# mmdagent/distantspeechrecognition-mirror

Measured on AMD Instinct MI355X. Metric: decoded_audio_hours_per_sec, higher is better.
Workload: dtype f32

## Files before the change

distantspeechrecognition-mirror_amd/csrc/decoder.cpp:

```cpp
#include "common.h"
#include "wfst_graph.h"
#include "lattice.h"
#include "lexicon.h"
#include "wordtrace.h"
#include "viterbi.h"
#include "decode_plan.h"
#include <algorithm>
#include <cmath>

namespace dsr {

static_assert(kPlanSideBytes == (size_t) kSideLds * sizeof(Side), "decode_plan.h budgets the side records of viterbi.h");

struct DecoderState {
  dsr_decoder_cfg cfg; bool haveGraph = false; int nSlots = 0; int nNodes = 0;
  WfstGraph::Csr csr; WfstGraph::Tables tab;
  DevBuf<int> d_xoff, d_xarc, d_xpathOff, d_eoff, d_path, d_nodeFinal, d_queue; DevBuf<float> d_pathCost;
  DevBuf<XRec> d_xrec; DevBuf<ERec> d_erec; DevBuf<float> d_arcCost, d_nodeCost; DevBuf<uint32_t> d_arcOut, d_arcIn;
  DevBuf<TokA> d_tokA, d_ctok; DevBuf<TokB> d_tokB; DevBuf<Side> d_side; DevBuf<XRecD> d_xrecD; int fastOK = 0; int maxCnt = 0; DevBuf<int> d_tokOff, d_tokCnt, d_owner, d_rank, d_chead; DevBuf<unsigned> d_tags; DevBuf<CandA> d_cA; DevBuf<CandB> d_cB; DevBuf<unsigned> d_first; DevBuf<Bp> d_arena;
  DevBuf<long long> d_prof; DevBuf<dsr_decode_result> d_res; DevBuf<int> d_arcs; DevBuf<unsigned> d_words;
  long arenaCap = 0; int initial = 0; unsigned tokenMemoryLimit = 0;
  long lastPoolCap = 0;
  hipEvent_t evTrace = nullptr;
  DevBuf<TraceHead> d_heads; DevBuf<int> d_hopRec, d_hopOff;
  DevBuf<SegState> d_segState; DevBuf<int> d_segDone; DevBuf<unsigned long long> d_poolNext; DevBuf<TokA> d_saveA; DevBuf<TokB> d_saveB;
  DevBuf<WTok> w_tok; DevBuf<WCand> w_cand; DevBuf<int> w_tokOff, w_rank; DevBuf<unsigned long long> w_best; DevBuf<unsigned> w_first; DevBuf<int4> w_traces; size_t w_tablesFor = 0;
  bool costNegZero = false; double costMinAbs = HUGE_VAL;
  DevBuf<uint4> d_lat; DevBuf<double> d_latTtl; DevBuf<long> d_latFrameOff; DevBuf<int> d_arenaLat; DevBuf<int4> d_latFinal; DevBuf<int> d_latInfo;
  int latU = 0, latTmax = 0; long latArenaCap = 0; WfstGraph graphCopy; DevBuf<TokA> d_tokA3; DevBuf<TokB> d_tokB3;
  const dsr_lexicon* lexIn = nullptr; const dsr_lexicon* lexOut = nullptr; uint32_t eosX = 0; std::string eosSymbol;
  int lastU = 0; size_t lastMaxPath = 0; bool lastPaths = false;
  PinBuf<dsr_decode_result> h_res; PinBuf<int> h_arcs; PinBuf<unsigned> h_words; hipEvent_t evDone = nullptr;
  int pendingU = 0; size_t pendingPath = 0; int pendingSlots = 0; long long* pendingProf = nullptr;
  int dumpOn = 0; long dumpCap = 0; DevBuf<long> d_dumpFrameOff, d_dumpCount; DevBuf<int> d_dumpNode, d_dumpArc; DevBuf<float> d_dumpAc, d_dumpLm;
  std::vector<int64_t> h_dumpFrameOff; std::vector<int32_t> h_dumpNode, h_dumpArc; std::vector<float> h_dumpAc, h_dumpLm; int64_t h_dumpFrames = 0;
};

}

using namespace dsr;
struct dsr_decoder : DecoderState {};

// ... 49 lines not shown

void dsr_decoder_destroy(dsr_decoder* d)
{
  if (!d) return;
  forget_traceback(d);
  if (d->evDone) (void) hipEventDestroy(d->evDone);
  if (d->evTrace) (void) hipEventDestroy(d->evTrace);
  delete d;
}

dsr_status dsr_decoder_set(dsr_decoder* d, const dsr_wfst* g)
{
  return guard([&] {
    if (!d || !g) throw Error(DSR_E_PARAMETER, "null argument");
    if (g->initial < 0) throw Error(DSR_E_CONSISTENCY, "the transducer has no arcs");
    d->csr = g->csr(); d->tab = g->tables(d->csr, (size_t) 1 << 28);
    d->nNodes = (int) g->nodes.size(); d->initial = g->initial; d->graphCopy = *g;
    std::vector<int> nf(d->nNodes); std::vector<float> nc(d->nNodes);
    for (int i = 0; i < d->nNodes; i++) { nf[i] = g->nodes[i].final_; nc[i] = g->nodes[i].cost; }
    d->d_xoff.upload(d->tab.xoff); d->d_eoff.upload(d->tab.eoff); d->d_path.upload(d->tab.path);
    if (d->tab.xrec.empty()) throw Error(DSR_E_CONSISTENCY, "the transducer has no emitting arcs");
    d->d_xrec.upload(d->tab.xrec); d->d_xarc.upload(d->tab.xarc); d->d_xpathOff.upload(d->tab.xpathOff);
    {
      const size_t nx = d->tab.xrec.size(); std::vector<XRecD> xd(nx); int maxCnt = 0; std::vector<float> pc(1, 0.0f);
      for (size_t r = 0; r < nx; r++) {
        const XRec& x = d->tab.xrec[r]; XRecD& o = xd[r];
        o.dst = x.dst; o.dist = x.dist; o.cost = x.cost; o.meta = x.meta; o.dstXoff = d->tab.xoff[x.dst]; o.dstCnt = d->tab.xoff[x.dst + 1] - d->tab.xoff[x.dst];
        const int po = d->tab.xpathOff[r], plen = (int) (x.meta & 0xFFFFu); o.p2 = 0; o.eps1 = 0.0f;
        if (x.meta >> 18) throw Error(DSR_E_CONSISTENCY, "expansion record %zu: meta bits above 17 are in use", r);
        if (plen) { const int a0 = d->tab.path[po]; o.eps1 = d->csr.cost[a0]; if (d->csr.out[a0] != 0) o.meta |= 0x20000u; }
        if (plen > 14) o.meta |= 0x80000000u;
        else if (plen > 1) {
          if (plen == 2) { const float c1 = d->csr.cost[d->tab.path[po + 1]]; memcpy(&o.p2, &c1, 4); }
          else { o.p2 = (int) pc.size(); for (int h = 1; h < plen; h++) pc.push_back(d->csr.cost[d->tab.path[po + h]]); }
          for (int h = 1; h < plen; h++) if (d->csr.out[d->tab.path[po + h]] != 0) o.meta |= 1u << (17 + h);
        }
        if (o.dstCnt > maxCnt) maxCnt = o.dstCnt;
      }
      d->d_xrecD.upload(xd); d->d_pathCost.upload(pc);
      d->fastOK = (maxCnt < (1 << 19) && nx < ((size_t) 1 << 27)) ? 1 : 0; d->maxCnt = maxCnt;
      if (read_vit_env().noFast) d->fastOK = 0;
    }
    { std::vector<ERec> e = d->tab.erec; if (e.empty()) e.push_back(ERec{0, 0, 0, 0}); d->d_erec.upload(e); }
    d->d_arcCost.upload(d->csr.cost); d->d_arcOut.upload(d->csr.out); d->d_arcIn.upload(d->csr.in);
    d->costNegZero = false; d->costMinAbs = HUGE_VAL;
    for (size_t a = 0; a < d->csr.cost.size(); a++) {
      const float c = d->csr.cost[a]; uint32_t bits; memcpy(&bits, &c, 4);
      if (bits == 0x80000000u) d->costNegZero = true;
      if (c != 0.0f && std::fabs((double) c) < d->costMinAbs) d->costMinAbs = std::fabs((double) c);
    }
    d->d_nodeFinal.upload(nf); d->d_nodeCost.upload(nc);
    d->haveGraph = true; d->nSlots = 0;
  });
}
dsr_status dsr_decoder_set_symbols(dsr_decoder* d, const dsr_wfst* g, const char* silSymbol, const char* eosSymbol)
{
  return guard([&] {
    if (!d || !g) throw Error(DSR_E_PARAMETER, "null argument");
    uint32_t silX = d->cfg.silenceX, eosX = 0;
    if (silSymbol) { if (!g->lexIn) throw Error(DSR_E_KEY, "the transducer has no input lexicon to look '%s' up in", silSymbol); silX = g->lexIn->index(silSymbol); }
    if (eosSymbol) { if (!g->lexOut) throw Error(DSR_E_KEY, "the transducer has no output lexicon to look '%s' up in", eosSymbol); eosX = g->lexOut->index(eosSymbol); }
    const dsr_status s = dsr_decoder_set(d, g);
// ... 145 lines not shown
  A.maxTok = c.maxActive; A.maxCand = c.maxCandidates; A.maxTraces = maxTraces;
  A.tok = d->w_tok.p; A.cand = d->w_cand.p; A.tokOff = d->w_tokOff.p; A.rank = d->w_rank.p; A.bestKey = d->w_best.p; A.firstSlot = d->w_first.p; A.traces = d->w_traces.p; A.queue = d->d_queue.p;
  A.scores = score; A.nframes = nframes; A.U = U; A.Tmax = Tmax; A.nDist = nDist; A.res = d->d_res.p; A.arcsOut = d->d_arcs.p; A.wordsOut = d->d_words.p; A.maxPath = maxPath;
  wordtrace_launch(A, slots, st);
  enqueue_result_copies(d, U, want_paths ? (size_t) U * maxPath : 0, st);
  d->pendingSlots = slots; d->pendingProf = nullptr; d->latU = 0;
}

static VitArgs fill_vit_args(dsr_decoder* d, const DecodePlan& P, const VitEnv& env, const float* score, const int32_t* nframes, int U, int Tmax, int nDist,
                             int maxPath, bool wantPaths, hipStream_t st)
{
  const int slots = P.slots; const bool latOn = d->cfg.latticeTokens > 0;
  d->d_res.reserve(U);
  if (wantPaths) { d->d_arcs.reserve((size_t) U * (maxPath > 0 ? maxPath : 1)); d->d_words.reserve((size_t) U * (maxPath > 0 ? maxPath : 1)); }
  DSR_HIP(hipMemsetAsync(d->d_queue.p, 0, 8 * sizeof(int), st));
  d->d_heads.reserve(U); DSR_HIP(hipMemsetAsync(d->d_heads.p, 0xFF, sizeof(TraceHead) * (size_t) U, st));
  if (d->dumpOn) {
    d->dumpCap = (long) d->cfg.maxActive * 64 < (long) 1 << 26 ? (long) 1 << 24 : (long) 1 << 26;
    d->d_dumpFrameOff.reserve(Tmax + 2); d->d_dumpCount.reserve(2);
    d->d_dumpNode.reserve(d->dumpCap); d->d_dumpArc.reserve(d->dumpCap); d->d_dumpAc.reserve(d->dumpCap); d->d_dumpLm.reserve(d->dumpCap);
    DSR_HIP(hipMemsetAsync(d->d_dumpCount.p, 0, 2 * sizeof(long), st));
  }
  VitArgs A; GraphDev& G = A.G; DecDev& D = A.D;
  G.nNodes = d->nNodes; G.initial = d->initial; G.xoff = d->d_xoff.p; G.xrec = d->d_xrec.p; G.xrecD = d->d_xrecD.p; G.xarc = d->d_xarc.p;
  G.xpathOff = d->d_xpathOff.p; G.eoff = d->d_eoff.p; G.erec = d->d_erec.p; G.path = d->d_path.p; G.pathCost = d->d_pathCost.p; G.arcCost = d->d_arcCost.p;
  G.arcOut = d->d_arcOut.p; G.arcIn = d->d_arcIn.p; G.nodeFinal = d->d_nodeFinal.p; G.nodeCost = d->d_nodeCost.p;
  D.beam = d->cfg.beam; D.lmScale = d->cfg.lmScale; D.lmPenalty = d->cfg.lmPenalty; D.silPenalty = d->cfg.silPenalty;
  D.noPen = (d->cfg.lmScale > 0.0 && std::isfinite(d->cfg.lmScale) && d->cfg.lmScale * d->cfg.lmPenalty == 0.0 && d->cfg.lmScale * d->cfg.silPenalty == 0.0 &&
             !d->costNegZero && (d->costMinAbs == HUGE_VAL || d->cfg.lmScale * d->costMinAbs >= 0x1p-60) && !env.pen) ? 1 : 0;
  D.silenceX = d->cfg.silenceX; D.maxTok = d->cfg.maxActive; D.maxCand = d->cfg.maxCandidates; D.arenaCap = d->arenaCap;
  D.tokA = d->d_tokA.p; D.tokB = d->d_tokB.p; D.ctok = d->d_ctok.p; D.side = d->d_side.p; D.fastOK = d->fastOK; D.tokOff = d->d_tokOff.p; D.owner = d->d_owner.p; D.rank = d->d_rank.p; D.cA = d->d_cA.p; D.cB = d->d_cB.p;
  D.first = d->d_first.p; D.tags = d->d_tags.p; D.tokCnt = d->d_tokCnt.p; D.chead = d->d_chead.p; D.arena = d->d_arena.p; D.queue = d->d_queue.p;
  D.segDrop = env.segDrop; D.segQueues = P.segQueues; D.segFrames = P.segFrames; D.segCount = P.segCount;
  D.poolCap = 0; D.poolChunk = 0; D.poolNext = nullptr; D.segState = nullptr; D.segDone = nullptr; D.saveA = nullptr; D.saveB = nullptr;
  if (P.segFrames > 0) {
    d->d_segState.reserve(U); d->d_segDone.reserve(U); d->d_poolNext.reserve(1);
    d->d_saveA.reserve((size_t) U * d->cfg.maxActive); d->d_saveB.reserve((size_t) U * d->cfg.maxActive);
    DSR_HIP(hipMemsetAsync(d->d_segDone.p, 0, sizeof(int) * (size_t) U, st)); DSR_HIP(hipMemsetAsync(d->d_poolNext.p, 0, sizeof(unsigned long long), st));
    D.poolCap = (long) ((size_t) std::max(P.poolArenas, slots) * (size_t) d->arenaCap); if (D.poolCap > (long) 0xFFFFFFF0L) D.poolCap = (long) 0xFFFFFFF0L;
    D.poolChunk = std::min<long>(262144, std::max<long>(4096, D.poolCap / (4 * (long) U)));
    D.poolNext = d->d_poolNext.p; D.segState = d->d_segState.p; D.segDone = d->d_segDone.p; D.saveA = d->d_saveA.p; D.saveB = d->d_saveB.p;
  }
  d->lastPoolCap = D.poolCap;
  D.prof = nullptr;
  if (env.prof) { d->d_prof.reserve((size_t) slots * kProfN); D.prof = d->d_prof.p; }
  D.dumpOn = d->dumpOn; D.dumpCap = d->dumpCap; D.dumpFrameOff = d->d_dumpFrameOff.p; D.dumpNode = d->d_dumpNode.p; D.dumpAc = d->d_dumpAc.p;
  D.dumpLm = d->d_dumpLm.p; D.dumpArc = d->d_dumpArc.p; D.dumpCount = d->d_dumpCount.p;
  D.topN = d->cfg.topN > 0 ? d->cfg.topN : 0; D.tokA3 = nullptr; D.tokB3 = nullptr;
  if (D.topN > 0) { d->d_tokA3.reserve((size_t) slots * d->cfg.maxActive); d->d_tokB3.reserve((size_t) slots * d->cfg.maxActive); D.tokA3 = d->d_tokA3.p; D.tokB3 = d->d_tokB3.p; }
// ... 254 lines not shown
```

distantspeechrecognition-mirror_amd/csrc/k_viterbi.hip:

```cpp
#include "launch.h"
#include "viterbi.h"
#include <algorithm>
#include <cmath>
#include <type_traits>

namespace dsr {

static constexpr uint32_t kNone = 0xFFFFFFFFu;
static constexpr uint32_t kEndBit = 0x80000000u;
static constexpr int kWaves = kThreads / 64;
static constexpr int kFastK = 8;
static constexpr int kB = 2;
static constexpr int kFastE = 8190;
static constexpr int kP1 = 16;
static constexpr int kW = 4;

typedef const __attribute__((address_space(4))) VitArgs* KP;

__device__ __forceinline__ unsigned ld_u32(const unsigned* p) { return __hip_atomic_load(p, __ATOMIC_RELAXED, __HIP_MEMORY_SCOPE_AGENT); }
__device__ __forceinline__ int ld_i32(const int* p) { return __hip_atomic_load(p, __ATOMIC_RELAXED, __HIP_MEMORY_SCOPE_AGENT); }
__device__ __forceinline__ void st_u32(unsigned* p, unsigned v) { __hip_atomic_store(p, v, __ATOMIC_RELAXED, __HIP_MEMORY_SCOPE_AGENT); }
__device__ __forceinline__ void st_i32(int* p, int v) { __hip_atomic_store(p, v, __ATOMIC_RELAXED, __HIP_MEMORY_SCOPE_AGENT); }
__device__ __forceinline__ void st_u64_dev(void* p, unsigned long long v) { __hip_atomic_store(reinterpret_cast<unsigned long long*>(p), v, __ATOMIC_RELAXED, __HIP_MEMORY_SCOPE_AGENT); }
__device__ __forceinline__ unsigned long long ld_u64_dev(const void* p) { return __hip_atomic_load(reinterpret_cast<const unsigned long long*>(p), __ATOMIC_RELAXED, __HIP_MEMORY_SCOPE_AGENT); }
// ... 376 lines not shown
            return atomicExch(&hkey[h], 0x80000000u | (unsigned) sx);
          };
          auto chain_head = [&](const unsigned h) __attribute__((always_inline)) -> unsigned {
            if (NARROW) { const unsigned w = tab[h]; return (w & 0x80000000u) ? (0x80000000u | ((w >> 15) & 0xFFFFu)) : 0u; }
            return hkey[h];
          };
          auto locate = [&](const int k, int& rec, unsigned& ekk) __attribute__((always_inline)) {
            const int c = k * nthr + tq; const int grp = k * nw + wq;
            unsigned e = 0u; int j = 0;
            if (c < C) {
              const unsigned long long W = ((unsigned long long) s_bm[2 * grp + 1] << 32) | s_bm[2 * grp];
              const unsigned gb = s_gbase[grp]; const unsigned long long mine = W & ((2ull << lq) - 1ull);
              e = (gb & 0x1FFFu) + (unsigned) __popcll(mine) - 1u;
              j = mine ? lq - (63 - __clzll((long long) mine)) : lq + (int) (gb >> 13);
            }
            ekk = e; rec = j;
          };
          auto tokload = [&](float& ac, float& lm, int& rec, unsigned& ekk) __attribute__((always_inline)) {
            const TokA t = *at32<TokA>(ctk, ekk * 16u);
            ac = t.ac; lm = t.lm; rec += (int) (t.xs & 0x7FFFFFFFu); ekk |= (t.xs >> 31) << 29;
          };
          auto expandR = [&](auto NOPEN, const int g8, float* ac8, float* lm8, int* rec8, unsigned* ek8) __attribute__((always_inline)) {
            constexpr bool NP = decltype(NOPEN)::value;
            int4 xr[kB]; int2 xd[kB]; bool tsil[kB];
#pragma unroll
            for (int i = 0; i < kB; i++) { tsil[i] = (ek8[i] >> 29) & 1u; ek8[i] &= 0x1FFFu; }
#pragma unroll
            for (int i = 0; i < kB; i++) {
              xr[i] = *at32<int4>(xrecD, (uint32_t) rec8[i] * 32u); xd[i] = *at32<int2>(xrecD, (uint32_t) rec8[i] * 32u + 16u);
            }
            if (PROF) { asm volatile("s_waitcnt vmcnt(0)" ::: "memory"); TICK(28); }
#pragma unroll
            for (int i = 0; i < kB; i++) {
              const int c = (g8 + i) * nthr + tq;
              if (c < C) {
                const int xdist = xr[i].x; const float xcost = __int_as_float(xr[i].y); const uint32_t xmeta = (uint32_t) xr[i].z;
                const float e1 = __int_as_float(xr[i].w);
                const int plen = (int) (xmeta & 0xFFFFu);
                const double lm0 = (double) lm8[i];
                const bool has = plen != 0;
                double lmNode;
                {
                  double l = __dadd_rn(lm0, __dmul_rn(lmS, (double) e1));
                  if (!NP) {
                    const double l1 = __dadd_rn(l, lsPen); l = (xmeta & 0x20000u) ? l1 : l;
                    const double l2 = __dadd_rn(l, lsSil); l = (sil0 && (prevNull0 || !tsil[i])) ? l2 : l;
                  }
                  lmNode = has ? (double) (float) l : lm0;
                }
                const bool pnull = has ? false : prevNull0;
                const bool pinSil = has ? sil0 : tsil[i];
                if (plen > 1) {
                  if (!(xmeta & 0x80000000u)) {
                    float hc0 = 0.0f, hc1 = 0.0f, hc2 = 0.0f;
                    if (plen > 2) { const float* pc = pathCost + xd[i].y; hc0 = pc[0]; hc1 = pc[1]; hc2 = pc[(plen > 3) ? 2 : 1]; }
                    for (int h = 1; h < plen; h++) {
                      const float ch = (plen == 2) ? __int_as_float(xd[i].y) : (h == 1 ? hc0 : h == 2 ? hc1 : h == 3 ? hc2 : pathCost[xd[i].y + h - 1]);
                      double l = __dadd_rn(lmNode, __dmul_rn(lmS, (double) ch));
                      if (!NP && ((xmeta >> (17 + h)) & 1u)) l = __dadd_rn(l, lsPen);
                      lmNode = (double) (float) l;
                    }
                  } else {
                    const int* pp = ka->G.path + ka->G.xpathOff[rec8[i]];
                    for (int h = 1; h < plen; h++) {
                      const int a = pp[h];
                      double l = __dadd_rn(lmNode, __dmul_rn(lmS, (double) ka->G.arcCost[a]));
                      if (!NP && ka->G.arcOut[a] != 0) l = __dadd_rn(l, lsPen);
                      lmNode = (double) (float) l;
                    }
                  }
                }
                double lm = __dadd_rn(lmNode, __dmul_rn(lmS, (double) xcost));
                if (!NP) { const double lm1 = __dadd_rn(lm, lsPen); lm = (xmeta & 0x10000u) ? lm1 : lm; }
                const bool silArc = ((uint32_t) (xdist + 1) == silenceX);
                if (!NP) { const double lm2 = __dadd_rn(lm, lsSil); lm = (silArc && (pnull || !pinSil)) ? lm2 : lm; }
                float rowv;
                if (useLdsRow) { rowv = ((const lds_float_t*) srow)[xdist]; DSR_NO_MERGE(); } else rowv = rowG[xdist];
                const double ac = __dadd_rn((double) ac8[i], (double) rowv);
                const double ttl = __dadd_rn(ac, lm);
                *at32w<double>(ttlS, (uint32_t) c * 8u) = ttl; ac8[i] = (float) ac; lm8[i] = (float) lm; rec8[i] |= (silArc ? 0x40000000 : 0);
                if (ttl < locMin) locMin = ttl;
                locMag = fmaxf(locMag, __fadd_rn(fabsf(ac8[i]), fabsf(lm8[i])));
                if (PROF) { asm volatile("s_waitcnt vmcnt(0) lgkmcnt(0)" ::: "memory"); TICK(29); }
                const unsigned prod = (unsigned) xd[i].x * 2654435761u;
                if (!NARROW && nPass > 1 && (prod >> 31)) ek8[i] |= 1u << 27;
                else ek8[i] |= (table_insert((unsigned) xd[i].x, prod, c) << 13) | (1u << 28);
                if (PROF) { asm volatile("s_waitcnt lgkmcnt(0)" ::: "memory"); TICK(30); }
              }
            }
          };
          auto expand8 = [&](auto NOPEN, const int g8, float* ac8, float* lm8, int* rec8, unsigned* ek8) __attribute__((always_inline)) {
#pragma unroll
            for (int i = 0; i < kB; i++) locate(g8 + i, rec8[i], ek8[i]);
            if (PROF) { asm volatile("s_waitcnt lgkmcnt(0)" ::: "memory"); TICK(26); }
#pragma unroll
            for (int i = 0; i < kB; i++) tokload(ac8[i], lm8[i], rec8[i], ek8[i]);
            if (PROF) { asm volatile("s_waitcnt vmcnt(0)" ::: "memory"); TICK(27); }
            expandR(NOPEN, g8, ac8, lm8, rec8, ek8);
          };
          auto park_store = [&](const int kb, const float* oac, const float* olm, const int* orec, const unsigned* oek) __attribute__((always_inline)) {
#pragma unroll
            for (int i = 0; i < kB; i++) { const int c = (kb + i) * nthr + tq; if (c < C) ovf[c - kFastK * nthr] = make_uint4(__float_as_uint(oac[i]), __float_as_uint(olm[i]), (unsigned) orec[i], oek[i]); }
          };
          auto park_load = [&](const int kb, float* oac, float* olm, int* orec, unsigned* oek) __attribute__((always_inline)) {
#pragma unroll
            for (int i = 0; i < kB; i++) {
              int c = (kb + i) * nthr + tq; c = (c < C) ? c : kFastK * nthr;
              const uint4 v = ovf[c - kFastK * nthr];
              oac[i] = __uint_as_float(v.x); olm[i] = __uint_as_float(v.y); orec[i] = (int) v.z; oek[i] = v.w;
// ... 47 lines not shown
            }
          };
          auto fold_multi = [&](const int wslot0, const unsigned head, const float ac, const float lm) __attribute__((always_inline)) -> int {
            int wslot = wslot0, wIdx = -1; double fw = (double) __fadd_rn(ac, lm);
            for (;;) {
              int best = 0x7FFFFFFF, bi = -1, steps = 0;
              for (unsigned p = head; (p & 0x80000000u) && steps <= C; steps++) {
                const int pi = (int) (p & 0x7FFFFFFFu);
                int pc; double pt; unsigned pn;
                side_link(sideL, side, sideLds, pi, pc, pt, pn);
                if (pc > wslot && pc < best && pt < fw) { best = pc; bi = pi; }
                p = pn;
              }
              if (bi < 0) break;
              wslot = best; wIdx = bi;
              fw = (double) side_score(sideL, side, sideLds, bi);
            }
            return wIdx;
          };
          auto fold1 = [&](const int k, const int pass, float& ac, float& lm, int& rec, unsigned& ekk, unsigned* defer) __attribute__((always_inline)) {
            const bool mine = ((firstMask >> k) & 1ull) && !(ekk & 0x80000000u) && (ekk & (1u << 28)) && in_pass(ekk, pass);
            if (mine) {
              const unsigned head = chain_head((ekk >> 13) & ekBucket);
              ekk &= 0x1FFFu;
              if (head & 0x80000000u) {
                int wIdx = -1;
                const int hi = (int) (head & 0x7FFFFFFFu);
                unsigned hnext; double pt;
                { int cdummy; side_link(sideL, side, sideLds, hi, cdummy, pt, hnext); }
                if (!(hnext & 0x80000000u)) {
                  if (pt < (double) __fadd_rn(ac, lm)) wIdx = hi;
                } else if (defer) *defer = head;
                else wIdx = fold_multi(k * nthr + tq, head, ac, lm);
                if (wIdx >= 0) {
                  side_winner(sideL, side, sideLds, wIdx, ac, lm, rec);
                  ekk = 0x80000000u | (unsigned) wIdx;
                }
              }
            }
          };
          auto insert8 = [&](const int g8, const int* rec8, unsigned* ek8) __attribute__((always_inline)) {
            int xd[kB];
#pragma unroll
            for (int i = 0; i < kB; i++) xd[i] = ka->G.xrecD[rec8[i] & 0x3FFFFFFF].dst;
#pragma unroll
            for (int i = 0; i < kB; i++) {
              const int c = (g8 + i) * nthr + tq;
              if (c < C && (ek8[i] & (1u << 27)) && !(ek8[i] & 0x80000000u)) ek8[i] |= (table_insert((unsigned) xd[i], (unsigned) xd[i] * 2654435761u, c) << 13) | (1u << 28);
            }
          };
          for (int pass = 0; pass < nPass; pass++) {
            if (!NARROW && pass > 0) {
              __syncthreads();
              { uint4* h4 = reinterpret_cast<uint4*>(hkey); const int q4 = hashN >> 2;
                for (int i = tq; i < 2 * q4; i += nthr) { unsigned wv = (i < q4) ? 0u : 0xFFFFFFFFu; asm volatile("" : "+v"(wv)); h4[i] = make_uint4(wv, wv, wv, wv); }    }
              __syncthreads();
#pragma unroll
              for (int g8 = 0; g8 < kFastK; g8 += kB) if (g8 < K) insert8(g8, &qrec[g8], &ek[g8]);
              for (int kb = kFastK; kb < K; kb += kB) {
                float oac[kB], olm[kB]; int orec[kB]; unsigned oek[kB]; park_load(kb, oac, olm, orec, oek);
                insert8(kb, orec, oek); park_store(kb, oac, olm, orec, oek);
              }
              __syncthreads();
            }
            {
              unsigned later = 0u;
#pragma unroll
// ... 65 lines not shown
#pragma unroll
          for (int k = 0; k < kFastK; k++) if (k < K && ((firstMask >> k) & 1ull)) {
            const float sc1 = __fadd_rn(qac[k], qlm[k]);
            if (!prune || !((double) sc1 > threshNext)) keepMask |= 1ull << k;
          }
          for (int kb = kFastK; kb < K; kb += kB) {
            float oac[kB], olm[kB]; int orec[kB]; unsigned oek[kB]; park_load(kb, oac, olm, orec, oek);
#pragma unroll
            for (int i = 0; i < kB; i++) if (kb + i < K && ((firstMask >> (kb + i)) & 1ull)) {
              const float sc1 = __fadd_rn(oac[i], olm[i]);
              if (!prune || !((double) sc1 > threshNext)) keepMask |= 1ull << (kb + i);
            }
          }
          int allFirst = 0;
          for (int k = 0; k < K; k++) {
            const unsigned long long bal = __ballot((keepMask >> k) & 1ull);
            if (lq == 0) s_cnt[k * nw + wq] = __popcll(bal);
            allFirst += __popcll(__ballot((firstMask >> k) & 1ull));
          }
          if (lq == 0) s_waveTotE[wq] = allFirst;
          TICK(13);
          __syncthreads();
          TICK(14);
          {
            uint4* h4 = reinterpret_cast<uint4*>(hkey); const int q4 = hashN >> 2;
            for (int i = tq; i < 2 * q4; i += nthr) { unsigned wv = (NARROW || i < q4) ? 0u : 0xFFFFFFFFu; asm volatile("" : "+v"(wv)); h4[i] = make_uint4(wv, wv, wv, wv); }
          }
          if (wq == 0) {
            const int nG = K * nw;
            int a[6], tot = 0;
#pragma unroll
            for (int q = 0; q < 6; q++) { a[q] = (6 * lq + q < nG) ? s_cnt[6 * lq + q] : 0; tot += a[q]; }
            const int incl = wave_incl_scan(tot, lq); int run = incl - tot;
#pragma unroll
            for (int q = 0; q < 6; q++) { if (6 * lq + q < nG) s_cnt[6 * lq + q] = run; run += a[q]; }
            if (lq == 63) s_waveTot[0] = incl;
          }
          __syncthreads();
          TICK(6);
          numNew = uni(s_waveTot[0]);
          { const int a = (lq < nw) ? s_waveTotE[lq] : 0; numStat = __builtin_amdgcn_readlane(wave_incl_scan(a, lq), 63); }
          RELOAD();
          if (numNew > ka->D.maxTok || (segS > 0 ? arenaUsed : arenaOff) + numNew > ka->D.arenaCap) { status = DSR_E_ALLOCATION; break; }
          if (segS > 0 && arenaOff + numNew > chunkEnd) {
            const long need = numNew > ka->D.poolChunk ? (long) numNew : ka->D.poolChunk;
            __syncthreads();
            if (tid == 0) s_chunk = (long long) atomicAdd(ka->D.poolNext, (unsigned long long) need);
            __syncthreads();
            arenaOff = (long) s_chunk; chunkEnd = arenaOff + need;
            if (chunkEnd > ka->D.poolCap) { status = DSR_E_ALLOCATION; break; }
          }
          const XRecD* const xrecW = ka->G.xrecD; TokA* const outA = nxtA; TokB* const outB = nxtB; Bp* const outBp = arena + arenaOff;
          auto write4 = [&](auto NB, const int g4, const float* ac4, const float* lm4, const int* rec4, const unsigned* ek4) __attribute__((always_inline)) {
            constexpr int nb = decltype(NB)::value;
            int4 dx[nb]; uint32_t pv[nb];
#pragma unroll
            for (int i = 0; i < nb; i++) {
              const bool kp = (keepMask >> (g4 + i)) & 1ull;
              dx[i] = *reinterpret_cast<const int4*>(&xrecW[kp ? (rec4[i] & 0x3FFFFFFF) : 0].dst);
              const bool sw = kp && (ek4[i] & 0x80000000u) != 0u; const unsigned si = ek4[i] & 0x7FFFFFFFu;
              const uint32_t* pb = (sw && si >= (unsigned) sideLds) ? &side[si].prevBp : &ctk[(sw || !kp) ? 0u : (ek4[i] & 0x1FFFu)].bp;
              pv[i] = *pb;
              if (sw && si < (unsigned) sideLds) pv[i] = sideL[si].prevBp;
            }
#pragma unroll
            for (int i = 0; i < nb; i++) {
              const int k = g4 + i;
              if (k < K) {
                const bool isFirst = (keepMask >> k) & 1ull;
                const unsigned long long bal = __ballot(isFirst);
                if (isFirst) {
                  const int pos = numNew - 1 - (s_cnt[k * nw + wq] + __popcll(bal & ((1ull << lq) - 1ull)));
                  TokA na; na.ac = ac4[i]; na.lm = lm4[i]; na.bp = (uint32_t) (arenaOff + pos); na.xs = (uint32_t) dx[i].z | ((rec4[i] & 0x40000000) ? 0x80000000u : 0u);
                  TokB nb; nb.node = dx[i].x; nb.cnt = dx[i].w;
                  Bp bp; bp.prev = pv[i]; bp.rec = (uint32_t) (rec4[i] & 0x3FFFFFFF);
                  outA[pos] = na; outB[pos] = nb; outBp[pos] = bp;
                  if (pos < cntCap) cntL[pos] = (unsigned short) dx[i].w;
                }
              }
            }
          };
          const bool dense = numNew <= (hashN >> 1);
          if (dense) {
            uint4* const stage = reinterpret_cast<uint4*>(hkey);
            auto stage1 = [&](const int k, const float ac, const float lm, const int rec, const unsigned ekk) __attribute__((always_inline)) {
              const bool isFirst = (keepMask >> k) & 1ull;
              const unsigned long long bal = __ballot(isFirst);
              if (isFirst) stage[s_cnt[k * nw + wq] + __popcll(bal & ((1ull << lq) - 1ull))] = make_uint4(__float_as_uint(ac), __float_as_uint(lm), (unsigned) rec, ekk);
            };
#pragma unroll
            for (int k = 0; k < kFastK; k++) if (k < K) stage1(k, qac[k], qlm[k], qrec[k], ek[k]);
            for (int kb = kFastK; kb < K; kb += kB) {
              float oac[kB], olm[kB]; int orec[kB]; unsigned oek[kB]; park_load(kb, oac, olm, orec, oek);
#pragma unroll
              for (int i = 0; i < kB; i++) if (kb + i < K) stage1(kb + i, oac[i], olm[i], orec[i], oek[i]);
            }
            __syncthreads();
            TICK(21);
            const int q4 = hashN >> 2;
            const bool layNext = prune && numNew <= 4 * nthr;
            preC = -1;
            auto denseLoad = [&](const int f0, uint4* en, int4* dx, uint32_t* pv) __attribute__((always_inline)) {
#pragma unroll
              for (int i = 0; i < 2; i++) {
                const int f = f0 + i * nthr + tq; const bool on = f < numNew;
                en[i] = stage[on ? f : 0];
                if (on) { unsigned wv = (NARROW || f < q4) ? 0u : 0xFFFFFFFFu; asm volatile("" : "+v"(wv)); stage[f] = make_uint4(wv, wv, wv, wv); }
              }
#pragma unroll
              for (int i = 0; i < 2; i++) {
                const bool on = f0 + i * nthr + tq < numNew;
                dx[i] = *at32<int4>(xrecW, (on ? (en[i].z & 0x3FFFFFFFu) : 0u) * 32u + 16u);
                const bool sw = on && (en[i].w & 0x80000000u) != 0u; const unsigned si = en[i].w & 0x7FFFFFFFu;
                const uint32_t* pb = (sw && si >= (unsigned) sideLds) ? &side[si].prevBp : &ctk[(sw || !on) ? 0u : (en[i].w & 0x1FFFu)].bp;
                pv[i] = *pb;
                if (sw && si < (unsigned) sideLds) pv[i] = sideL[si].prevBp;
              }
            };
            auto denseStore = [&](const int f0, const uint4* en, const int4* dx, const uint32_t* pv) __attribute__((always_inline)) {
#pragma unroll
              for (int i = 0; i < 2; i++) {
                const int f = f0 + i * nthr + tq;
                if (f < numNew) {
                  const int pos = numNew - 1 - f;
                  TokA na; na.ac = __uint_as_float(en[i].x); na.lm = __uint_as_float(en[i].y); na.bp = (uint32_t) (arenaOff + pos); na.xs = (uint32_t) dx[i].z | ((en[i].z & 0x40000000u) ? 0x80000000u : 0u);
                  TokB nb; nb.node = dx[i].x; nb.cnt = dx[i].w;
                  Bp bp; bp.prev = pv[i]; bp.rec = (uint32_t) (en[i].z & 0x3FFFFFFFu);
                  outA[pos] = na; outB[pos] = nb; outBp[pos] = bp;
                  if (pos < cntCap) cntL[pos] = (unsigned short) dx[i].w;
                }
              }
            };
            auto layOut = [&](auto NE_, const int* cn) __attribute__((always_inline)) {
              constexpr int NE = decltype(NE_)::value;
              int in[NE]; bool bad = false;
#pragma unroll
              for (int i = 0; i < NE; i++) {
                in[i] = wave_incl_scan(cn[i], lq);
                bad = bad || (i * nthr + tq < numNew && cn[i] == 0);
              }
              const int badW = __any(bad) ? 1 : 0;
              if (lq == 63) {
#pragma unroll
                for (int i = 0; i < NE; i++) s_cnt[i * nw + wq] = in[i];
                s_waveTotE[wq] = badW;
              }
              __syncthreads();
              const int tg = (lq < NE * nw) ? s_cnt[lq] : 0;
              const int sg = wave_incl_scan(tg, lq);
              const int total = __builtin_amdgcn_readlane(sg, 63), wu = uni(wq);
              const bool anyBad = __any(((lq < nw) ? s_waveTotE[lq] : 0) != 0);
              const bool fits = total <= fastCapC;
#pragma unroll
              for (int i = 0; i < NE; i++) {
                const int f = i * nthr + tq; const int off = total - (__builtin_amdgcn_readlane(sg - tg, i * nw + wu) + in[i]);
                if (fits && f < numNew && cn[i] > 0) {
                  const int e = numNew - 1 - f;
                  atomicOr(&s_bm[off >> 5], 1u << (off & 31));
                  for (int g = (off >> 6) + 1; g <= ((off + cn[i]) >> 6); g++) s_gbase[g] = (unsigned) (e + 1) | ((unsigned) (64 * g - off) << 13);
                }
              }
              if (tq == 0) { s_sideN = 0; s_gbase[0] = 0; s_err = 0; }
              preC = (anyBad || !fits) ? -1 : total;
            };
            if (layNext && numNew > 2 * nthr) {
              int cn[4];
#pragma unroll
              for (int h = 0; h < 2; h++) {
                uint4 en[2]; int4 dx[2]; uint32_t pv[2];
                denseLoad(h * 2 * nthr, en, dx, pv); denseStore(h * 2 * nthr, en, dx, pv);
#pragma unroll
                for (int i = 0; i < 2; i++) cn[2 * h + i] = ((2 * h + i) * nthr + tq < numNew) ? dx[i].w : 0;
              }
              layOut(std::integral_constant<int, 4>{}, cn);
            } else {
              for (int f0 = 0; f0 < numNew; f0 += 2 * nthr) {
                uint4 en[2]; int4 dx[2]; uint32_t pv[2];
                denseLoad(f0, en, dx, pv);
                if (layNext) {
                  const int cn[2] = { (tq < numNew) ? dx[0].w : 0, (nthr + tq < numNew) ? dx[1].w : 0 };
                  layOut(std::integral_constant<int, 2>{}, cn);
                }
                denseStore(f0, en, dx, pv);
              }
            }
            TICK(22);
          } else
          {
#pragma unroll
          for (int g4 = 0; g4 < kFastK; g4 += kW) if (g4 < K) write4(std::integral_constant<int, kW>{}, g4, &qac[g4], &qlm[g4], &qrec[g4], &ek[g4]);
          for (int kb = kFastK; kb < K; kb += kB) {
            float oac[kB], olm[kB]; int orec[kB]; unsigned oek[kB]; park_load(kb, oac, olm, orec, oek);
            write4(std::integral_constant<int, kB>{}, kb, oac, olm, orec, oek);
          }
          TICK(21);
          TICK(22);
          preC = -1;
          }
          cntOK = prune && numNew <= cntCap;
        }
      }
      if (!fast) {
      cntOK = false; preC = -1;
// ... 364 lines not shown
```

distantspeechrecognition-mirror_amd/csrc/viterbi.h:

```cpp
#pragma once
#include "common.h"
#include "wfst_graph.h"

namespace dsr {

struct Tok { int32_t node; float ac; float lm; uint32_t bp; };
struct TokA { float ac; float lm; uint32_t bp; uint32_t xs; };
struct TokB { int32_t node; int32_t cnt; };
struct XRecD { int32_t dist; float cost; uint32_t meta; float eps1; int32_t dst; int32_t p2; int32_t dstXoff; int32_t dstCnt; };
struct Side { double ttl; float ac; float lm; int32_t rec; uint32_t prevBp; int32_t c; uint32_t next; };
struct CandA { double ttl; float ac; float lm; };
struct CandB { int32_t dst; int32_t next; int32_t rec; uint32_t prevBp; };
struct Bp { uint32_t prev; uint32_t rec; };
struct TraceHead { unsigned long long arenaOff; uint32_t bp; uint32_t hops; };
static_assert(sizeof(TokA) == 16 && sizeof(TokB) == 8 && sizeof(XRecD) == 32 && sizeof(Side) == 32 && sizeof(CandA) == 16 && sizeof(CandB) == 16 && sizeof(Bp) == 8 && sizeof(TraceHead) == 16,
              "record layouts shared by the host and k_viterbi");

static constexpr int kThreads = 1024;
static constexpr int kFastC = 24576;
static constexpr int kProfN = 48;
static constexpr int kSideLds = 496;

struct GraphDev {
  int nNodes, initial;
  const int* xoff; const XRec* xrec; const XRecD* xrecD; const int* xarc; const int* xpathOff;
  const int* eoff; const ERec* erec; const int* path; const float* pathCost;
  const float* arcCost; const uint32_t* arcOut; const uint32_t* arcIn;
  const int* nodeFinal; const float* nodeCost;
};

struct SegState { int n, status, maxActive, pad; long arenaOff, chunkEnd, arenaUsed; double thresh; long long stat[3]; };

struct DecDev {
  double beam, lmScale, lmPenalty, silPenalty; uint32_t silenceX; int noPen;
  int segFrames, segCount, segQueues, segDrop; long poolCap, poolChunk;    unsigned long long* poolNext; SegState* segState; int* segDone; TokA* saveA; TokB* saveB;
  int maxTok, maxCand; long arenaCap;
  TokA* tokA; TokB* tokB; TokA* ctok; Side* side; int fastOK; int* tokOff; int* tokCnt; int* owner; int* rank; int* chead; CandA* cA; CandB* cB; unsigned* first; unsigned* tags; Bp* arena;
  int* queue; long long* prof;
  int dumpOn; long dumpCap; long* dumpFrameOff; int* dumpNode; float* dumpAc; float* dumpLm; int* dumpArc; long* dumpCount;
  int latOn; long latCap; uint4* lat; double* latTtl; long* latFrameOff; int* arenaLat; int4* latFinal; int* latInfo;
  int topN; TokA* tokA3; TokB* tokB3;
};

struct VitArgs {
  GraphDev G; DecDev D;
  const float* scores; const int* nframesArr; int U, Tmax, nDist;
  dsr_decode_result* res; int* arcsOut; unsigned* wordsOut; int maxPath, useLdsRow, hashN, regionB, cntCap;
  TraceHead* heads;
// ... 18 lines not shown
```

Before: 27.13.

## Split expansion records into hot/cold structs and precompute lmScale-weighted costs

The 32-byte expansion record is split into an expansion part holding precomputed double lmScale*cost and lmScale*eps1 values, and a separate 16-byte record with dst/dstXoff/dstCnt used by the insert and write phases. This removes two double multiplies per candidate and halves the bytes fetched in the token-write path. The hash table clear in the narrow mode is replaced by zeroing each used bucket on consumption. lmScale is now frozen at graph-set time, and the decoder throws if it changes afterwards.

```diff
diff --git a/distantspeechrecognition-mirror_amd/csrc/decoder.cpp b/distantspeechrecognition-mirror_amd/csrc/decoder.cpp
--- a/distantspeechrecognition-mirror_amd/csrc/decoder.cpp
+++ b/distantspeechrecognition-mirror_amd/csrc/decoder.cpp
@@ -17,7 +17,7 @@
   WfstGraph::Csr csr; WfstGraph::Tables tab;
   DevBuf<int> d_xoff, d_xarc, d_xpathOff, d_eoff, d_path, d_nodeFinal, d_queue; DevBuf<float> d_pathCost;
   DevBuf<XRec> d_xrec; DevBuf<ERec> d_erec; DevBuf<float> d_arcCost, d_nodeCost; DevBuf<uint32_t> d_arcOut, d_arcIn;
-  DevBuf<TokA> d_tokA, d_ctok; DevBuf<TokB> d_tokB; DevBuf<Side> d_side; DevBuf<XRecD> d_xrecD; int fastOK = 0; int maxCnt = 0; DevBuf<int> d_tokOff, d_tokCnt, d_owner, d_rank, d_chead; DevBuf<unsigned> d_tags; DevBuf<CandA> d_cA; DevBuf<CandB> d_cB; DevBuf<unsigned> d_first; DevBuf<Bp> d_arena;
+  DevBuf<TokA> d_tokA, d_ctok; DevBuf<TokB> d_tokB; DevBuf<Side> d_side; DevBuf<XRecD> d_xrecD; DevBuf<XRecC> d_xrecC; double recLmScale = 0.0;  int fastOK = 0; int maxCnt = 0; DevBuf<int> d_tokOff, d_tokCnt, d_owner, d_rank, d_chead; DevBuf<unsigned> d_tags; DevBuf<CandA> d_cA; DevBuf<CandB> d_cB; DevBuf<unsigned> d_first; DevBuf<Bp> d_arena;
   DevBuf<long long> d_prof; DevBuf<dsr_decode_result> d_res; DevBuf<int> d_arcs; DevBuf<unsigned> d_words;
   long arenaCap = 0; int initial = 0; unsigned tokenMemoryLimit = 0;
   long lastPoolCap = 0;
@@ -113,22 +113,25 @@
     if (d->tab.xrec.empty()) throw Error(DSR_E_CONSISTENCY, "the transducer has no emitting arcs");
     d->d_xrec.upload(d->tab.xrec); d->d_xarc.upload(d->tab.xarc); d->d_xpathOff.upload(d->tab.xpathOff);
     {
-      const size_t nx = d->tab.xrec.size(); std::vector<XRecD> xd(nx); int maxCnt = 0; std::vector<float> pc(1, 0.0f);
+      const size_t nx = d->tab.xrec.size(); std::vector<XRecD> xd(nx); std::vector<XRecC> xc(nx); int maxCnt = 0; std::vector<float> pc(1, 0.0f);
+      const double lmS = d->cfg.lmScale; d->recLmScale = lmS;
       for (size_t r = 0; r < nx; r++) {
-        const XRec& x = d->tab.xrec[r]; XRecD& o = xd[r];
-        o.dst = x.dst; o.dist = x.dist; o.cost = x.cost; o.meta = x.meta; o.dstXoff = d->tab.xoff[x.dst]; o.dstCnt = d->tab.xoff[x.dst + 1] - d->tab.xoff[x.dst];
-        const int po = d->tab.xpathOff[r], plen = (int) (x.meta & 0xFFFFu); o.p2 = 0; o.eps1 = 0.0f;
+        const XRec& x = d->tab.xrec[r]; XRecD& o = xd[r]; XRecC& oc = xc[r];
+        o.dst = x.dst; o.dist = x.dist; o.lmCost = lmS * (double) x.cost; o.meta = x.meta;
+        oc.dst = x.dst; oc.dstXoff = d->tab.xoff[x.dst]; oc.dstCnt = d->tab.xoff[x.dst + 1] - d->tab.xoff[x.dst]; oc.pad = 0;
+        const int po = d->tab.xpathOff[r], plen = (int) (x.meta & 0xFFFFu); o.p2 = 0; float eps1 = 0.0f;
         if (x.meta >> 18) throw Error(DSR_E_CONSISTENCY, "expansion record %zu: meta bits above 17 are in use", r);
-        if (plen) { const int a0 = d->tab.path[po]; o.eps1 = d->csr.cost[a0]; if (d->csr.out[a0] != 0) o.meta |= 0x20000u; }
+        if (plen) { const int a0 = d->tab.path[po]; eps1 = d->csr.cost[a0]; if (d->csr.out[a0] != 0) o.meta |= 0x20000u; }
+        o.lmEps1 = lmS * (double) eps1;
         if (plen > 14) o.meta |= 0x80000000u;
         else if (plen > 1) {
           if (plen == 2) { const float c1 = d->csr.cost[d->tab.path[po + 1]]; memcpy(&o.p2, &c1, 4); }
           else { o.p2 = (int) pc.size(); for (int h = 1; h < plen; h++) pc.push_back(d->csr.cost[d->tab.path[po + h]]); }
           for (int h = 1; h < plen; h++) if (d->csr.out[d->tab.path[po + h]] != 0) o.meta |= 1u << (17 + h);
         }
-        if (o.dstCnt > maxCnt) maxCnt = o.dstCnt;
+        if (oc.dstCnt > maxCnt) maxCnt = oc.dstCnt;
       }
-      d->d_xrecD.upload(xd); d->d_pathCost.upload(pc);
+      d->d_xrecD.upload(xd); d->d_xrecC.upload(xc); d->d_pathCost.upload(pc);
       d->fastOK = (maxCnt < (1 << 19) && nx < ((size_t) 1 << 27)) ? 1 : 0; d->maxCnt = maxCnt;
       if (read_vit_env().noFast) d->fastOK = 0;
     }
@@ -320,9 +323,10 @@
     DSR_HIP(hipMemsetAsync(d->d_dumpCount.p, 0, 2 * sizeof(long), st));
   }
   VitArgs A; GraphDev& G = A.G; DecDev& D = A.D;
-  G.nNodes = d->nNodes; G.initial = d->initial; G.xoff = d->d_xoff.p; G.xrec = d->d_xrec.p; G.xrecD = d->d_xrecD.p; G.xarc = d->d_xarc.p;
+  G.nNodes = d->nNodes; G.initial = d->initial; G.xoff = d->d_xoff.p; G.xrec = d->d_xrec.p; G.xrecD = d->d_xrecD.p; G.xrecC = d->d_xrecC.p; G.xarc = d->d_xarc.p;
   G.xpathOff = d->d_xpathOff.p; G.eoff = d->d_eoff.p; G.erec = d->d_erec.p; G.path = d->d_path.p; G.pathCost = d->d_pathCost.p; G.arcCost = d->d_arcCost.p;
   G.arcOut = d->d_arcOut.p; G.arcIn = d->d_arcIn.p; G.nodeFinal = d->d_nodeFinal.p; G.nodeCost = d->d_nodeCost.p;
+  if (memcmp(&d->recLmScale, &d->cfg.lmScale, sizeof(double)) != 0) throw Error(DSR_E_CONSISTENCY, "lmScale changed after the transducer was set");
   D.beam = d->cfg.beam; D.lmScale = d->cfg.lmScale; D.lmPenalty = d->cfg.lmPenalty; D.silPenalty = d->cfg.silPenalty;
   D.noPen = (d->cfg.lmScale > 0.0 && std::isfinite(d->cfg.lmScale) && d->cfg.lmScale * d->cfg.lmPenalty == 0.0 && d->cfg.lmScale * d->cfg.silPenalty == 0.0 &&
              !d->costNegZero && (d->costMinAbs == HUGE_VAL || d->cfg.lmScale * d->costMinAbs >= 0x1p-60) && !env.pen) ? 1 : 0;
diff --git a/distantspeechrecognition-mirror_amd/csrc/k_viterbi.hip b/distantspeechrecognition-mirror_amd/csrc/k_viterbi.hip
--- a/distantspeechrecognition-mirror_amd/csrc/k_viterbi.hip
+++ b/distantspeechrecognition-mirror_amd/csrc/k_viterbi.hip
@@ -422,40 +422,38 @@
           };
           auto expandR = [&](auto NOPEN, const int g8, float* ac8, float* lm8, int* rec8, unsigned* ek8) __attribute__((always_inline)) {
             constexpr bool NP = decltype(NOPEN)::value;
-            int4 xr[kB]; int2 xd[kB]; bool tsil[kB];
-#pragma unroll
-            for (int i = 0; i < kB; i++) { tsil[i] = (ek8[i] >> 29) & 1u; ek8[i] &= 0x1FFFu; }
+            int4 xr[kB]; double2 xl[kB];
 #pragma unroll
             for (int i = 0; i < kB; i++) {
-              xr[i] = *at32<int4>(xrecD, (uint32_t) rec8[i] * 32u); xd[i] = *at32<int2>(xrecD, (uint32_t) rec8[i] * 32u + 16u);
+              xr[i] = *at32<int4>(xrecD, (uint32_t) rec8[i] * 32u); xl[i] = *at32<double2>(xrecD, (uint32_t) rec8[i] * 32u + 16u);
             }
             if (PROF) { asm volatile("s_waitcnt vmcnt(0)" ::: "memory"); TICK(28); }
 #pragma unroll
             for (int i = 0; i < kB; i++) {
               const int c = (g8 + i) * nthr + tq;
+              const bool tsil = (ek8[i] >> 29) & 1u; ek8[i] &= 0x1FFFu;
               if (c < C) {
-                const int xdist = xr[i].x; const float xcost = __int_as_float(xr[i].y); const uint32_t xmeta = (uint32_t) xr[i].z;
-                const float e1 = __int_as_float(xr[i].w);
+                const int xdist = xr[i].x; const uint32_t xmeta = (uint32_t) xr[i].y; const int xdst = xr[i].z, xp2 = xr[i].w;
                 const int plen = (int) (xmeta & 0xFFFFu);
                 const double lm0 = (double) lm8[i];
                 const bool has = plen != 0;
                 double lmNode;
                 {
-                  double l = __dadd_rn(lm0, __dmul_rn(lmS, (double) e1));
+                  double l = __dadd_rn(lm0, xl[i].y);
                   if (!NP) {
                     const double l1 = __dadd_rn(l, lsPen); l = (xmeta & 0x20000u) ? l1 : l;
-                    const double l2 = __dadd_rn(l, lsSil); l = (sil0 && (prevNull0 || !tsil[i])) ? l2 : l;
+                    const double l2 = __dadd_rn(l, lsSil); l = (sil0 && (prevNull0 || !tsil)) ? l2 : l;
                   }
                   lmNode = has ? (double) (float) l : lm0;
                 }
                 const bool pnull = has ? false : prevNull0;
-                const bool pinSil = has ? sil0 : tsil[i];
+                const bool pinSil = has ? sil0 : tsil;
                 if (plen > 1) {
                   if (!(xmeta & 0x80000000u)) {
                     float hc0 = 0.0f, hc1 = 0.0f, hc2 = 0.0f;
-                    if (plen > 2) { const float* pc = pathCost + xd[i].y; hc0 = pc[0]; hc1 = pc[1]; hc2 = pc[(plen > 3) ? 2 : 1]; }
+                    if (plen > 2) { const float* pc = pathCost + xp2; hc0 = pc[0]; hc1 = pc[1]; hc2 = pc[(plen > 3) ? 2 : 1]; }
                     for (int h = 1; h < plen; h++) {
-                      const float ch = (plen == 2) ? __int_as_float(xd[i].y) : (h == 1 ? hc0 : h == 2 ? hc1 : h == 3 ? hc2 : pathCost[xd[i].y + h - 1]);
+                      const float ch = (plen == 2) ? __int_as_float(xp2) : (h == 1 ? hc0 : h == 2 ? hc1 : h == 3 ? hc2 : pathCost[xp2 + h - 1]);
                       double l = __dadd_rn(lmNode, __dmul_rn(lmS, (double) ch));
                       if (!NP && ((xmeta >> (17 + h)) & 1u)) l = __dadd_rn(l, lsPen);
                       lmNode = (double) (float) l;
@@ -470,7 +468,7 @@
                     }
                   }
                 }
-                double lm = __dadd_rn(lmNode, __dmul_rn(lmS, (double) xcost));
+                double lm = __dadd_rn(lmNode, xl[i].x);
                 if (!NP) { const double lm1 = __dadd_rn(lm, lsPen); lm = (xmeta & 0x10000u) ? lm1 : lm; }
                 const bool silArc = ((uint32_t) (xdist + 1) == silenceX);
                 if (!NP) { const double lm2 = __dadd_rn(lm, lsSil); lm = (silArc && (pnull || !pinSil)) ? lm2 : lm; }
@@ -482,9 +480,9 @@
                 if (ttl < locMin) locMin = ttl;
                 locMag = fmaxf(locMag, __fadd_rn(fabsf(ac8[i]), fabsf(lm8[i])));
                 if (PROF) { asm volatile("s_waitcnt vmcnt(0) lgkmcnt(0)" ::: "memory"); TICK(29); }
-                const unsigned prod = (unsigned) xd[i].x * 2654435761u;
+                const unsigned prod = (unsigned) xdst * 2654435761u;
                 if (!NARROW && nPass > 1 && (prod >> 31)) ek8[i] |= 1u << 27;
-                else ek8[i] |= (table_insert((unsigned) xd[i].x, prod, c) << 13) | (1u << 28);
+                else ek8[i] |= (table_insert((unsigned) xdst, prod, c) << 13) | (1u << 28);
                 if (PROF) { asm volatile("s_waitcnt lgkmcnt(0)" ::: "memory"); TICK(30); }
               }
             }
@@ -578,6 +576,7 @@
             const bool mine = ((firstMask >> k) & 1ull) && !(ekk & 0x80000000u) && (ekk & (1u << 28)) && in_pass(ekk, pass);
             if (mine) {
               const unsigned head = chain_head((ekk >> 13) & ekBucket);
+              if (NARROW) tab[(ekk >> 13) & ekBucket] = 0u;
               ekk &= 0x1FFFu;
               if (head & 0x80000000u) {
                 int wIdx = -1;
@@ -598,7 +597,7 @@
           auto insert8 = [&](const int g8, const int* rec8, unsigned* ek8) __attribute__((always_inline)) {
             int xd[kB];
 #pragma unroll
-            for (int i = 0; i < kB; i++) xd[i] = ka->G.xrecD[rec8[i] & 0x3FFFFFFF].dst;
+            for (int i = 0; i < kB; i++) xd[i] = ka->G.xrecC[rec8[i] & 0x3FFFFFFF].dst;
 #pragma unroll
             for (int i = 0; i < kB; i++) {
               const int c = (g8 + i) * nthr + tq;
@@ -710,9 +709,9 @@
           TICK(13);
           __syncthreads();
           TICK(14);
-          {
+          if (!NARROW) {
             uint4* h4 = reinterpret_cast<uint4*>(hkey); const int q4 = hashN >> 2;
-            for (int i = tq; i < 2 * q4; i += nthr) { unsigned wv = (NARROW || i < q4) ? 0u : 0xFFFFFFFFu; asm volatile("" : "+v"(wv)); h4[i] = make_uint4(wv, wv, wv, wv); }
+            for (int i = tq; i < 2 * q4; i += nthr) { unsigned wv = (i < q4) ? 0u : 0xFFFFFFFFu; asm volatile("" : "+v"(wv)); h4[i] = make_uint4(wv, wv, wv, wv); }
           }
           if (wq == 0) {
             const int nG = K * nw;
@@ -738,14 +737,14 @@
             arenaOff = (long) s_chunk; chunkEnd = arenaOff + need;
             if (chunkEnd > ka->D.poolCap) { status = DSR_E_ALLOCATION; break; }
           }
-          const XRecD* const xrecW = ka->G.xrecD; TokA* const outA = nxtA; TokB* const outB = nxtB; Bp* const outBp = arena + arenaOff;
+          const XRecC* const xrecW = ka->G.xrecC; TokA* const outA = nxtA; TokB* const outB = nxtB; Bp* const outBp = arena + arenaOff;
           auto write4 = [&](auto NB, const int g4, const float* ac4, const float* lm4, const int* rec4, const unsigned* ek4) __attribute__((always_inline)) {
             constexpr int nb = decltype(NB)::value;
             int4 dx[nb]; uint32_t pv[nb];
 #pragma unroll
             for (int i = 0; i < nb; i++) {
               const bool kp = (keepMask >> (g4 + i)) & 1ull;
-              dx[i] = *reinterpret_cast<const int4*>(&xrecW[kp ? (rec4[i] & 0x3FFFFFFF) : 0].dst);
+              dx[i] = *reinterpret_cast<const int4*>(&xrecW[kp ? (rec4[i] & 0x3FFFFFFF) : 0]);
               const bool sw = kp && (ek4[i] & 0x80000000u) != 0u; const unsigned si = ek4[i] & 0x7FFFFFFFu;
               const uint32_t* pb = (sw && si >= (unsigned) sideLds) ? &side[si].prevBp : &ctk[(sw || !kp) ? 0u : (ek4[i] & 0x1FFFu)].bp;
               pv[i] = *pb;
@@ -759,11 +758,11 @@
                 const unsigned long long bal = __ballot(isFirst);
                 if (isFirst) {
                   const int pos = numNew - 1 - (s_cnt[k * nw + wq] + __popcll(bal & ((1ull << lq) - 1ull)));
-                  TokA na; na.ac = ac4[i]; na.lm = lm4[i]; na.bp = (uint32_t) (arenaOff + pos); na.xs = (uint32_t) dx[i].z | ((rec4[i] & 0x40000000) ? 0x80000000u : 0u);
-                  TokB nb; nb.node = dx[i].x; nb.cnt = dx[i].w;
+                  TokA na; na.ac = ac4[i]; na.lm = lm4[i]; na.bp = (uint32_t) (arenaOff + pos); na.xs = (uint32_t) dx[i].y | ((rec4[i] & 0x40000000) ? 0x80000000u : 0u);
+                  TokB nb; nb.node = dx[i].x; nb.cnt = dx[i].z;
                   Bp bp; bp.prev = pv[i]; bp.rec = (uint32_t) (rec4[i] & 0x3FFFFFFF);
                   outA[pos] = na; outB[pos] = nb; outBp[pos] = bp;
-                  if (pos < cntCap) cntL[pos] = (unsigned short) dx[i].w;
+                  if (pos < cntCap) cntL[pos] = (unsigned short) dx[i].z;
                 }
               }
             }
@@ -798,7 +797,7 @@
 #pragma unroll
               for (int i = 0; i < 2; i++) {
                 const bool on = f0 + i * nthr + tq < numNew;
-                dx[i] = *at32<int4>(xrecW, (on ? (en[i].z & 0x3FFFFFFFu) : 0u) * 32u + 16u);
+                dx[i] = *at32<int4>(xrecW, (on ? (en[i].z & 0x3FFFFFFFu) : 0u) * 16u);
                 const bool sw = on && (en[i].w & 0x80000000u) != 0u; const unsigned si = en[i].w & 0x7FFFFFFFu;
                 const uint32_t* pb = (sw && si >= (unsigned) sideLds) ? &side[si].prevBp : &ctk[(sw || !on) ? 0u : (en[i].w & 0x1FFFu)].bp;
                 pv[i] = *pb;
@@ -811,11 +810,11 @@
                 const int f = f0 + i * nthr + tq;
                 if (f < numNew) {
                   const int pos = numNew - 1 - f;
-                  TokA na; na.ac = __uint_as_float(en[i].x); na.lm = __uint_as_float(en[i].y); na.bp = (uint32_t) (arenaOff + pos); na.xs = (uint32_t) dx[i].z | ((en[i].z & 0x40000000u) ? 0x80000000u : 0u);
-                  TokB nb; nb.node = dx[i].x; nb.cnt = dx[i].w;
+                  TokA na; na.ac = __uint_as_float(en[i].x); na.lm = __uint_as_float(en[i].y); na.bp = (uint32_t) (arenaOff + pos); na.xs = (uint32_t) dx[i].y | ((en[i].z & 0x40000000u) ? 0x80000000u : 0u);
+                  TokB nb; nb.node = dx[i].x; nb.cnt = dx[i].z;
                   Bp bp; bp.prev = pv[i]; bp.rec = (uint32_t) (en[i].z & 0x3FFFFFFFu);
                   outA[pos] = na; outB[pos] = nb; outBp[pos] = bp;
-                  if (pos < cntCap) cntL[pos] = (unsigned short) dx[i].w;
+                  if (pos < cntCap) cntL[pos] = (unsigned short) dx[i].z;
                 }
               }
             };
@@ -858,7 +857,7 @@
                 uint4 en[2]; int4 dx[2]; uint32_t pv[2];
                 denseLoad(h * 2 * nthr, en, dx, pv); denseStore(h * 2 * nthr, en, dx, pv);
 #pragma unroll
-                for (int i = 0; i < 2; i++) cn[2 * h + i] = ((2 * h + i) * nthr + tq < numNew) ? dx[i].w : 0;
+                for (int i = 0; i < 2; i++) cn[2 * h + i] = ((2 * h + i) * nthr + tq < numNew) ? dx[i].z : 0;
               }
               layOut(std::integral_constant<int, 4>{}, cn);
             } else {
@@ -866,7 +865,7 @@
                 uint4 en[2]; int4 dx[2]; uint32_t pv[2];
                 denseLoad(f0, en, dx, pv);
                 if (layNext) {
-                  const int cn[2] = { (tq < numNew) ? dx[0].w : 0, (nthr + tq < numNew) ? dx[1].w : 0 };
+                  const int cn[2] = { (tq < numNew) ? dx[0].z : 0, (nthr + tq < numNew) ? dx[1].z : 0 };
                   layOut(std::integral_constant<int, 2>{}, cn);
                 }
                 denseStore(f0, en, dx, pv);
diff --git a/distantspeechrecognition-mirror_amd/csrc/viterbi.h b/distantspeechrecognition-mirror_amd/csrc/viterbi.h
--- a/distantspeechrecognition-mirror_amd/csrc/viterbi.h
+++ b/distantspeechrecognition-mirror_amd/csrc/viterbi.h
@@ -7,13 +7,14 @@
 struct Tok { int32_t node; float ac; float lm; uint32_t bp; };
 struct TokA { float ac; float lm; uint32_t bp; uint32_t xs; };
 struct TokB { int32_t node; int32_t cnt; };
-struct XRecD { int32_t dist; float cost; uint32_t meta; float eps1; int32_t dst; int32_t p2; int32_t dstXoff; int32_t dstCnt; };
+struct XRecD { int32_t dist; uint32_t meta; int32_t dst; int32_t p2; double lmCost; double lmEps1; };
+struct XRecC { int32_t dst; int32_t dstXoff; int32_t dstCnt; int32_t pad; };
 struct Side { double ttl; float ac; float lm; int32_t rec; uint32_t prevBp; int32_t c; uint32_t next; };
 struct CandA { double ttl; float ac; float lm; };
 struct CandB { int32_t dst; int32_t next; int32_t rec; uint32_t prevBp; };
 struct Bp { uint32_t prev; uint32_t rec; };
 struct TraceHead { unsigned long long arenaOff; uint32_t bp; uint32_t hops; };
-static_assert(sizeof(TokA) == 16 && sizeof(TokB) == 8 && sizeof(XRecD) == 32 && sizeof(Side) == 32 && sizeof(CandA) == 16 && sizeof(CandB) == 16 && sizeof(Bp) == 8 && sizeof(TraceHead) == 16,
+static_assert(sizeof(TokA) == 16 && sizeof(TokB) == 8 && sizeof(XRecD) == 32 && sizeof(XRecC) == 16 && sizeof(Side) == 32 && sizeof(CandA) == 16 && sizeof(CandB) == 16 && sizeof(Bp) == 8 && sizeof(TraceHead) == 16,
               "record layouts shared by the host and k_viterbi");
 
 static constexpr int kThreads = 1024;
@@ -23,7 +24,7 @@
 
 struct GraphDev {
   int nNodes, initial;
-  const int* xoff; const XRec* xrec; const XRecD* xrecD; const int* xarc; const int* xpathOff;
+  const int* xoff; const XRec* xrec; const XRecD* xrecD; const XRecC* xrecC; const int* xarc; const int* xpathOff;
   const int* eoff; const ERec* erec; const int* path; const float* pathCost;
   const float* arcCost; const uint32_t* arcOut; const uint32_t* arcIn;
   const int* nodeFinal; const float* nodeCost;
```

Result: faster. 27.80, median of 6 (+2.4%).
